# isarandi/metrabs

Hardware: AMD Instinct MI355X
Metric: crops/sec (256px, 72 depth bins) at 1/2/4/8 MI355X; MPJPE vs ref (higher is better)
Workload: dtype f32

## Files before the change

### include/metrabs_hip.h

```cpp
#ifndef METRABS_HIP_H_
#define METRABS_HIP_H_

#include <stddef.h>
#include <stdint.h>

#ifdef __cplusplus
extern "C" {
#endif

#define MTR_VERSION 100

typedef void* mtr_stream_t;

enum mtr_dtype { MTR_F32 = 0, MTR_F16 = 1, MTR_BF16 = 2 };

enum mtr_layout {
  MTR_NCHW = 0,
  MTR_NHWC = 1
};

enum mtr_error {
  MTR_OK = 0,
  MTR_E_NULL = -1,
  MTR_E_SHAPE = -2,
// ... 178 lines not shown
int mtr_bias_act_nchw(void* y, int dtype, const float* bias , const void* residual, int act,
                      long long B, int C, int HW, mtr_stream_t stream);

int mtr_bias_act_rowmean_nchw(void* y, int dtype, const float* bias , int act, long long B,
                              int C, int HW, float* row_mean , mtr_stream_t stream);

int mtr_depthwise3x3_bias_act(const void* x, int dtype, const float* weight, const float* bias, int act,
                              long long B, int C, int H, int W, int stride, int pad, void* y,
                              float* row_mean, mtr_stream_t stream);
int mtr_depthwise3x3_bias_act_padded(const void* x, int dtype, const float* weight, const float* bias,
                                     int act, long long B, int C, int H, int W, int stride, int pad_top,
                                     int pad_left, int pad_bottom, int pad_right, void* y,
                                     float* row_mean, mtr_stream_t stream);

int mtr_depthwise5x5_bias_act_padded(const void* x, int dtype, const float* weight ,
                                     const float* bias, int act, long long B, int C, int H, int W,
                                     int stride, int pad_top, int pad_left, int pad_bottom, int pad_right,
                                     void* y, float* row_mean , mtr_stream_t stream);

int mtr_se_gate(const float* mean , const float* w1, const float* b1, const float* w2,
                const float* b2, int act, int gate_fn, int B, int C, int S, float* gate ,
                mtr_stream_t stream);

int mtr_conv1x1_bias_act(const void* x, int dtype, const float* weight, const float* bias,
                         const float* gate , const void* residual, int act, long long B,
                         int M, int K, int HW, void* y, mtr_stream_t stream);

int mtr_conv1x1_bias_act16(const void* x, int dtype, const void* weight, const float* bias,
                           const float* gate , const void* residual, int act, long long B,
                           int M, int K, int HW, void* y, mtr_stream_t stream);

int mtr_conv3x3_bias_act16(const void* x, int dtype, const void* weight , const float* bias,
                           const void* residual, int act, long long B, int Cin, int Cout, int H, int W, int stride,
                           void* y, mtr_stream_t stream);

size_t mtr_conv3x3_16_lds_bytes(long long B, int Cin, int Cout, int H, int W, int stride);

#ifdef __cplusplus
}
#endif
#endif
```

### metrabs_amd/_lib.py

```python
import ctypes
import os
from ctypes import POINTER, c_char_p, c_double, c_float, c_int, c_int32, c_size_t, c_uint8, c_void_p

LIB_PATH = os.path.join(os.path.dirname(os.path.abspath(__file__)), 'csrc', 'libmetrabs_hip.so')

MTR_F32, MTR_F16, MTR_BF16 = 0, 1, 2
MTR_NCHW, MTR_NHWC = 0, 1
MTR_WARP_PARAM_FLOATS = 36


class HeadParams(ctypes.Structure):
    _fields_ = [('proc_side', c_int32), ('stride_test', c_int32), ('centered_stride', c_int32),
                ('legacy_centered_stride_bug', c_int32), ('box_size_mm', c_float)]


class HeadOptions(ctypes.Structure):
    _fields_ = [('struct_size', ctypes.c_uint32),
                ('rt_tiles_per_workgroup', c_int32), ('groups_per_workgroup', c_int32),
                ('dma_staging', c_int32), ('rt_column_blocks', c_int32), ('rt_k_groups', c_int32),
                ('rt_loader', c_int32), ('rt_split_column_blocks', c_int32)]


def head_options(rt_tiles=0, groups_per_workgroup=0, dma_staging=-1, rt_column_blocks=0, rt_k_groups=0,
                 rt_loader=0, rt_split=0):
# ... 92 lines not shown
    'mtr_detector_preprocess': (c_int, [c_void_p, c_int, c_int, c_int, POINTER(DetectorGeom), c_void_p,
                                        c_void_p]),
    'mtr_detector_preprocess_kernel': (c_int, [c_void_p, c_int, c_int, c_int, POINTER(DetectorGeom), c_int,
                                               c_void_p, c_void_p]),
    'mtr_detector_scale_boxes': (c_int, [c_void_p, c_int, POINTER(DetectorGeom), c_void_p, c_void_p]),
    'mtr_filter_poses_workspace_bytes': (ctypes.c_size_t, [c_int, c_int, c_int]),
    'mtr_filter_poses': (c_int, [c_void_p, c_void_p, c_void_p, c_void_p, c_void_p, c_int, c_int, c_int,
                                 c_int, c_void_p, c_void_p, c_int, c_int, POINTER(FilterParams), c_void_p,
                                 ctypes.c_size_t, c_int, c_void_p, c_void_p, c_void_p, c_void_p]),
    'mtr_depthwise3x3_bias_act': (c_int, [c_void_p, c_int, c_void_p, c_void_p, c_int, ctypes.c_longlong,
                                          c_int, c_int, c_int, c_int, c_int, c_void_p, c_void_p, c_void_p]),
    'mtr_depthwise3x3_bias_act_padded': (c_int, [c_void_p, c_int, c_void_p, c_void_p, c_int, ctypes.c_longlong,
                                                 c_int, c_int, c_int, c_int, c_int, c_int, c_int, c_int,
                                                 c_void_p, c_void_p, c_void_p]),
    'mtr_depthwise5x5_bias_act_padded': (c_int, [c_void_p, c_int, c_void_p, c_void_p, c_int, ctypes.c_longlong,
                                                 c_int, c_int, c_int, c_int, c_int, c_int, c_int, c_int,
                                                 c_void_p, c_void_p, c_void_p]),
    'mtr_bias_act_rowmean_nchw': (c_int, [c_void_p, c_int, c_void_p, c_int, ctypes.c_longlong, c_int, c_int,
                                          c_void_p, c_void_p]),
    'mtr_bias_act_nchw': (c_int, [c_void_p, c_int, c_void_p, c_void_p, c_int, ctypes.c_longlong, c_int,
                                  c_int, c_void_p]),
    'mtr_se_gate': (c_int, [c_void_p, c_void_p, c_void_p, c_void_p, c_void_p, c_int, c_int, c_int, c_int,
                            c_int, c_void_p, c_void_p]),
    'mtr_conv1x1_bias_act': (c_int, [c_void_p, c_int, c_void_p, c_void_p, c_void_p, c_void_p, c_int,
                                     ctypes.c_longlong, c_int, c_int, c_int, c_void_p, c_void_p]),
    'mtr_conv1x1_bias_act16': (c_int, [c_void_p, c_int, c_void_p, c_void_p, c_void_p, c_void_p, c_int,
                                       ctypes.c_longlong, c_int, c_int, c_int, c_void_p, c_void_p]),
    'mtr_conv3x3_bias_act16': (c_int, [c_void_p, c_int, c_void_p, c_void_p, c_void_p, c_int, ctypes.c_longlong,
                                       c_int, c_int, c_int, c_int, c_int, c_void_p, c_void_p]),
    'mtr_conv3x3_16_lds_bytes': (ctypes.c_size_t, [ctypes.c_longlong, c_int, c_int, c_int, c_int, c_int]),
}

_lib = None


def load(path=None):
    global _lib
    if _lib is not None and path is None:
        return _lib
    path = path or LIB_PATH
    import torch
    if not os.path.exists(path):
        raise RuntimeError(
            f'{path} not found: the HIP extension is not built. Run `python -m metrabs_amd.build` '
            f'(needs hipcc). metrabs_amd has no CPU fallback.')
    lib = ctypes.CDLL(path)
# ... 34 lines not shown
```

### metrabs_amd/backbones.py

```python
import collections
import threading

import torch
import torch.nn.functional as F
from torch import nn


class DepthwiseConv2d(nn.Conv2d):

    use_miopen = False
    _backend_lock = threading.Lock()

    def forward(self, x):
        if x.is_cuda and not DepthwiseConv2d.use_miopen and torch.backends.cudnn.enabled:
            cudnn = torch.backends.cudnn
            with DepthwiseConv2d._backend_lock, cudnn.flags(
                    enabled=False, benchmark=cudnn.benchmark, deterministic=cudnn.deterministic,
                    allow_tf32=cudnn.allow_tf32):
                return super().forward(x)
        return super().forward(x)


class ConvBNAct(nn.Sequential):

# ... 6 lines not shown
            layers.append(act())
        super().__init__(*layers)


class SqueezeExcite(nn.Module):
    def __init__(self, channels, squeeze, gate=nn.Sigmoid, act=nn.SiLU):
        super().__init__()
        self.fc1 = nn.Conv2d(channels, squeeze, 1)
        self.fc2 = nn.Conv2d(squeeze, channels, 1)
        self.act, self.gate = act(), gate()

    mean_from = ()
    gate_to = ()

    _GATE_NAMES = {nn.Sigmoid: 'sigmoid', nn.Hardsigmoid: 'hardsigmoid'}

    def forward(self, x):
        mean = None
        for src in self.mean_from:
            mean = src.take_mean_f32(x)
        if mean is not None and self._fused_gate_ok():
            from . import kernels
            g = kernels.se_gate(mean, self.fc1.weight, self.fc1.bias, self.fc2.weight, self.fc2.bias,
                                _ACT_NAMES[type(self.act)], self._GATE_NAMES[type(self.gate)])
            for dst in self.gate_to:
                if dst.k13_takes(x) or dst.k13h_takes(x):
                    dst.give_gate(x, g)
                    return x
            return x * g.to(x.dtype).view(x.shape[0], x.shape[1], 1, 1)
        if x.dtype != self.fc1.weight.dtype and not torch.is_autocast_enabled(x.device.type):
            return self._forward_16bit_copy(x, mean)
        s = None if mean is None else mean.to(x.dtype).view(x.shape[0], x.shape[1], 1, 1)
        if s is None:
            s = x.mean((2, 3), keepdim=True)
        return x * self.gate(self.fc2(self.act(self.fc1(s))))

    def _forward_16bit_copy(self, x, mean):
        s = mean.view(x.shape[0], x.shape[1], 1, 1) if mean is not None else \
            x.mean((2, 3), keepdim=True, dtype=self.fc1.weight.dtype)
        return x * self.gate(self.fc2(self.act(self.fc1(s)))).to(x.dtype)

    def _fused_gate_ok(self):
        if torch.is_grad_enabled() and any(p.requires_grad for p in self.parameters()):
            return False
        return (type(self.act) in (nn.SiLU, nn.ReLU) and type(self.gate) in self._GATE_NAMES
                and self.fc1.weight.dtype == torch.float32 and self.fc1.bias is not None
                and self.fc2.bias is not None and self.fc1.weight.is_cuda
                and self.fc1.in_channels % 4 == 0)


def _padded_conv(layers, name, cin, cout, k, stride, groups=1, act=nn.SiLU, bottomright=False):
    total = k - 1
    beg, end = total // 2, total - total // 2
    if bottomright:
        layers['padding'] = nn.ZeroPad2d((beg - 1, end + 1, beg - 1, end + 1))
        layers[name] = ConvBNAct(cin, cout, k, stride, groups=groups, act=act, padding=0)
    elif beg == end:
        layers[name] = ConvBNAct(cin, cout, k, stride, groups=groups, act=act, padding=beg)
    else:
        layers['padding'] = nn.ZeroPad2d((beg, end, beg, end))
        layers[name] = ConvBNAct(cin, cout, k, stride, groups=groups, act=act, padding=0)


# ... 136 lines not shown
        return resnet18()
    if name in ('mobilenetv3', 'mobilenetv3-large', 'mobilenet-v3'):
        return mobilenet_v3_large()
    raise ValueError(f'unknown backbone {name}')


_ACT_NAMES = {nn.SiLU: 'silu', nn.ReLU: 'relu', nn.Hardswish: 'hardswish'}


class ConvBiasAct(nn.Module):

    def __init__(self, conv, bias, act):
        super().__init__()
        self.conv = conv
        self.register_buffer('bias', bias.detach().float().contiguous())
        self.act = act
        self.act_name = None if act is None else _ACT_NAMES[type(act)]
        self.emit_mean = False
        self._mean = None
        self._gate = None
        self.last_path = None

    use_k13 = True
    k13_slower = frozenset({(960, 256, 64), (1536, 256, 64), (256, 1280, 64)})

    def k13_takes(self, x):
        c = self.conv
        if not (ConvBiasAct.use_k13 and not self.emit_mean and x.is_cuda and c.kernel_size == (1, 1)
                and c.stride == (1, 1) and c.padding == (0, 0) and c.dilation == (1, 1) and c.groups == 1
                and c.bias is None and c.padding_mode == 'zeros'):
            return False
        if torch.is_autocast_enabled('cuda') or (torch.is_grad_enabled() and c.weight.requires_grad):
            return False
        if x.dim() != 4 or (c.in_channels, c.out_channels, x.shape[2] * x.shape[3]) in ConvBiasAct.k13_slower:
            return False
        from . import kernels
        return kernels.conv1x1_supported(x, c.weight)

    use_k13h = True
    k13h_slower = frozenset({(192, 48, 4096), (256, 64, 1024), (1536, 256, 64), (256, 64, 9216), (768, 192, 576),
                             (1152, 224, 576), (1344, 224, 576), (1344, 384, 144), (2304, 384, 144),
                             (2304, 640, 144), (640, 3840, 144), (3840, 640, 144), (640, 1280, 144)})

    def k13h_takes(self, x):
        c = self.conv
        if not (ConvBiasAct.use_k13h and not self.emit_mean and x.is_cuda and x.dtype == c.weight.dtype
                and x.dtype in (torch.float16, torch.bfloat16) and c.kernel_size == (1, 1)
# ... 269 lines not shown
```

### metrabs_amd/csrc/conv1x1.hip

```cpp
#include "common.h"

namespace mtr {

typedef float f32x16 __attribute__((ext_vector_type(16)));

constexpr int kC1PadX = 32;
constexpr int kC1PadW = 4;

template <int WM, int WN, int FM, int FN, int BK, int ACT>
__global__ __launch_bounds__(64 * WM * WN) void conv1x1_kernel(
    const float* __restrict__ x, const float* __restrict__ w, const float* __restrict__ bias,
    const float* __restrict__ gate, const float* __restrict__ residual, float* __restrict__ y, int M,
    int K, int HW, int n_total, FastDiv by_hw) {
  constexpr int NT = 64 * WM * WN;
  constexpr int BM = 32 * FM * WM, BN = 32 * FN * WN;
  constexpr int LDX = BN + kC1PadX, LDW = BM + kC1PadW;
  constexpr int XROW4 = BN / 4;
  constexpr int XPASS = NT / XROW4;
  constexpr int XV = (BK + XPASS - 1) / XPASS;
  constexpr int WPASS = NT / (BK / 4);
  constexpr int WV = (BM + WPASS - 1) / WPASS;
  static_assert(NT % XROW4 == 0 && NT % (BK / 4) == 0, "loader mapping");
  __shared__ float xs[2][BK * LDX];
  __shared__ float ws[2][BK * LDW];
// ... 92 lines not shown
#pragma unroll
    for (int j = 0; j < FN; ++j) {
#pragma unroll
      for (int g = 0; g < 4; ++g) {
        const int col = n0 + wn * (32 * FN) + j * 32 + 8 * g + 4 * half;
        if (col >= n_total) continue;
        const unsigned b = fastdiv((unsigned)col, by_hw);
        const long long off = ((long long)b * M + m) * HW + (col - (int)b * HW);
        float4 r;
        r.x = activate<ACT>(acc[i][j][4 * g + 0] + bm);
        r.y = activate<ACT>(acc[i][j][4 * g + 1] + bm);
        r.z = activate<ACT>(acc[i][j][4 * g + 2] + bm);
        r.w = activate<ACT>(acc[i][j][4 * g + 3] + bm);
        if (residual) {
          const float4 q = *reinterpret_cast<const float4*>(residual + off);
          r.x += q.x; r.y += q.y; r.z += q.z; r.w += q.w;
        }
        *reinterpret_cast<float4*>(y + off) = r;
      }
    }
  }
}

enum Conv1x1Config { kCfgWide = 0, kCfgSquare = 1, kCfgTall = 2 };

struct Conv1x1Plan { int cfg, waves_m, bm, bn; };

inline Conv1x1Plan pick_config(int M, int K, int HW, long long B) {
  const long long n_total = B * HW;
  const long long n_tiles128 = (n_total + 127) / 128;
  if (M <= 160) {
    const int w = (M + 31) / 32;
    return {kCfgTall, w, 32 * w, 32};
  }
  if (M == 256 && K >= 512) return {kCfgTall, 4, 128, 32};
  if (M % 192 == 0 && (M / 192) * n_tiles128 >= 512) return {kCfgWide, 2, 192, 128};
  return {kCfgSquare, 2, 128, 128};
}

template <int WM, int WN, int FM, int FN, int BK>
static int launch_conv1x1_cfg(const float* x, const float* w, const float* bias, const float* gate,
                              const float* residual, float* y, int act, int M, int K, int HW,
                              long long n_total, hipStream_t stream) {
  constexpr int BM = 32 * FM * WM, BN = 32 * FN * WN;
  const long long gx = (n_total + BN - 1) / BN, gy = (M + BM - 1) / BM;
  if (gx > 0x7fffffffLL || gy > 65535) return MTR_E_SHAPE;
  const dim3 grid((unsigned)gx, (unsigned)gy), block(64 * WM * WN);
  const FastDiv by_hw = make_fastdiv((unsigned)HW);
  MTR_CLEAR_STALE();
#define MTR_C1_LAUNCH(ACT)                                                                                    \
  hipLaunchKernelGGL((conv1x1_kernel<WM, WN, FM, FN, BK, ACT>), grid, block, 0, stream, x, w, bias, gate, residual, \
                     y, M, K, HW, (int)n_total, by_hw)
  switch (act) {
    case kActNone: MTR_C1_LAUNCH(kActNone); break;
    case kActRelu: MTR_C1_LAUNCH(kActRelu); break;
    case kActSilu: MTR_C1_LAUNCH(kActSilu); break;
    case kActHardswish: MTR_C1_LAUNCH(kActHardswish); break;
    default: return MTR_E_PARAM;
  }
#undef MTR_C1_LAUNCH
  MTR_CHECK_LAUNCH();
  return MTR_OK;
}

}

extern "C" int mtr_conv1x1_bias_act(const void* x, int dtype, const float* weight, const float* bias,
                                    const float* gate, const void* residual, int act, long long B, int M,
                                    int K, int HW, void* y, mtr_stream_t stream) {
  if (!x || !weight || !bias || !y) return MTR_E_NULL;
  if (dtype != MTR_F32) return MTR_E_DTYPE;
  if (B < 0 || M <= 0 || K <= 0 || HW <= 0) return MTR_E_SHAPE;
  if (HW % 4 || K % 4) return MTR_E_SHAPE;
  if (B * HW > 0x7fffffffLL || (long long)K * HW > 0x7fffffffLL || (long long)M * HW > 0x7fffffffLL)
    return MTR_E_SHAPE;
  if (act < mtr::kActNone || act > mtr::kActHardswish) return MTR_E_PARAM;
  if (((uintptr_t)x % 16) || ((uintptr_t)weight % 16) || ((uintptr_t)y % 16) || ((uintptr_t)residual % 16))
    return MTR_E_ALIGN;
  if (x == y || (residual && residual == x)) return MTR_E_PARAM;
  if (B == 0) return MTR_OK;
  const float* xf = (const float*)x;
  const float* rf = (const float*)residual;
  float* yf = (float*)y;
  const long long n_total = B * HW;
  hipStream_t s = (hipStream_t)stream;
  const mtr::Conv1x1Plan p = mtr::pick_config(M, K, HW, B);
  switch (p.cfg) {
    case mtr::kCfgWide:
      return mtr::launch_conv1x1_cfg<2, 2, 3, 2, 16>(xf, weight, bias, gate, rf, yf, act, M, K, HW, n_total, s);
    case mtr::kCfgSquare:
      return mtr::launch_conv1x1_cfg<2, 2, 2, 2, 16>(xf, weight, bias, gate, rf, yf, act, M, K, HW, n_total, s);
    default:
      switch (p.waves_m) {
        case 1: return mtr::launch_conv1x1_cfg<1, 1, 1, 1, 16>(xf, weight, bias, gate, rf, yf, act, M, K, HW, n_total, s);
        case 2: return mtr::launch_conv1x1_cfg<2, 1, 1, 1, 16>(xf, weight, bias, gate, rf, yf, act, M, K, HW, n_total, s);
        case 3: return mtr::launch_conv1x1_cfg<3, 1, 1, 1, 16>(xf, weight, bias, gate, rf, yf, act, M, K, HW, n_total, s);
        case 4: return mtr::launch_conv1x1_cfg<4, 1, 1, 1, 32>(xf, weight, bias, gate, rf, yf, act, M, K, HW, n_total, s);
        default: return mtr::launch_conv1x1_cfg<5, 1, 1, 1, 16>(xf, weight, bias, gate, rf, yf, act, M, K, HW, n_total, s);
      }
  }
}
```

### metrabs_amd/csrc/se.hip

```cpp
#include "common.h"

namespace mtr {

enum SeGate { kGateSigmoid = 0, kGateHardsigmoid = 1 };

constexpr int kSeThreads = 256;
constexpr int kSeImg = 4;
constexpr int kSeRows = 4;
constexpr int kSeUnroll = 4;

template <int ACT, int GATE>
__global__ __launch_bounds__(kSeThreads) void se_gate_kernel(const float* __restrict__ mean,
                                                             const float* __restrict__ w1,
                                                             const float* __restrict__ b1,
                                                             const float* __restrict__ w2,
                                                             const float* __restrict__ b2, int B,
                                                             int C, int S, float* __restrict__ gate) {
  extern __shared__ float4 se_lds[];
  const int C4 = C >> 2;
  float4* m_tile = se_lds;
  float* hid = reinterpret_cast<float*>(se_lds + kSeImg * C4);
  const int b0 = blockIdx.y * kSeImg;
  const int tid = threadIdx.x, lane = tid & 63, wave = tid >> 6;

  for (int i = tid; i < kSeImg * C4; i += kSeThreads) {
    const int img = i / C4, c4 = i - img * C4;
    m_tile[i] = b0 + img < B ? reinterpret_cast<const float4*>(mean)[(long long)(b0 + img) * C4 + c4]
                             : make_float4(0.0f, 0.0f, 0.0f, 0.0f);
  }
  __syncthreads();

  const int n_blocks = (S + kSeRows - 1) / kSeRows;
  for (int blk = wave; blk < n_blocks; blk += kSeThreads / 64) {
    const float4* wrow[kSeRows];
#pragma unroll
    for (int r = 0; r < kSeRows; ++r) {
      const int s = min(blk * kSeRows + r, S - 1);
      wrow[r] = reinterpret_cast<const float4*>(w1 + (long long)s * C);
    }
    float acc[kSeRows][kSeImg];
#pragma unroll
    for (int r = 0; r < kSeRows; ++r)
#pragma unroll
      for (int i = 0; i < kSeImg; ++i) acc[r][i] = 0.0f;
    for (int c0 = lane; c0 < C4; c0 += 64 * kSeUnroll) {
      float4 w[kSeUnroll][kSeRows];
#pragma unroll
      for (int u = 0; u < kSeUnroll; ++u)
#pragma unroll
        for (int r = 0; r < kSeRows; ++r)
          w[u][r] = wrow[r][min(c0 + 64 * u, C4 - 1)];
#pragma unroll
      for (int u = 0; u < kSeUnroll; ++u) {
        const int c4 = c0 + 64 * u;
        const bool live = c4 < C4;
        float4 m[kSeImg];
#pragma unroll
        for (int i = 0; i < kSeImg; ++i) {
          const float4 v = m_tile[i * C4 + min(c4, C4 - 1)];
          m[i] = live ? v : make_float4(0.0f, 0.0f, 0.0f, 0.0f);
        }
#pragma unroll
        for (int r = 0; r < kSeRows; ++r)
#pragma unroll
          for (int i = 0; i < kSeImg; ++i) {
            float a = acc[r][i];
            a = fmaf(w[u][r].x, m[i].x, a);
            a = fmaf(w[u][r].y, m[i].y, a);
            a = fmaf(w[u][r].z, m[i].z, a);
            a = fmaf(w[u][r].w, m[i].w, a);
            acc[r][i] = a;
          }
      }
    }
#pragma unroll
    for (int r = 0; r < kSeRows; ++r)
#pragma unroll
      for (int i = 0; i < kSeImg; ++i) {
        float v = acc[r][i];
#pragma unroll
        for (int k = 32; k >= 1; k >>= 1) v += __shfl_xor(v, k, 64);
        acc[r][i] = v;
      }
    if (lane == 0) {
#pragma unroll
      for (int r = 0; r < kSeRows; ++r) {
        const int s = blk * kSeRows + r;
        if (s < S) {
#pragma unroll
          for (int i = 0; i < kSeImg; ++i) hid[i * S + s] = activate<ACT>(acc[r][i] + b1[s]);
        }
      }
    }
  }
  __syncthreads();

  const int c = blockIdx.x * kSeThreads + tid;
  if (c >= C) return;
  const float* w2row = w2 + (long long)c * S;
  float z[kSeImg];
#pragma unroll
  for (int i = 0; i < kSeImg; ++i) z[i] = 0.0f;
#pragma unroll 16
  for (int s = 0; s < S; ++s) {
    const float w = w2row[s];
#pragma unroll
    for (int i = 0; i < kSeImg; ++i) z[i] = fmaf(w, hid[i * S + s], z[i]);
  }
  const float bias = b2[c];
#pragma unroll
  for (int i = 0; i < kSeImg; ++i) {
    if (b0 + i >= B) break;
    const float x = z[i] + bias;
    float g;
    if constexpr (GATE == kGateSigmoid) g = 1.0f / (1.0f + expf(-x));
    else g = fminf(fmaxf(x + 3.0f, 0.0f), 6.0f) / 6.0f;
    gate[(long long)(b0 + i) * C + c] = g;
  }
}

template <int ACT>
static int launch_se_gate(const float* mean, const float* w1, const float* b1, const float* w2,
                          const float* b2, int gate_fn, int B, int C, int S, float* gate,
                          hipStream_t stream) {
  const size_t lds = (size_t)kSeImg * C * sizeof(float) + (size_t)kSeImg * S * sizeof(float);
  const dim3 grid((C + kSeThreads - 1) / kSeThreads, (B + kSeImg - 1) / kSeImg), block(kSeThreads);
  const void* kern = gate_fn == kGateSigmoid ? (const void*)se_gate_kernel<ACT, kGateSigmoid>
                                             : (const void*)se_gate_kernel<ACT, kGateHardsigmoid>;
  if (lds > 64 * 1024) {
    const int e = allow_dynamic_lds(kern, lds);
    if (e != MTR_OK) return e;
  }
  MTR_CLEAR_STALE();
  if (gate_fn == kGateSigmoid)
    hipLaunchKernelGGL((se_gate_kernel<ACT, kGateSigmoid>), grid, block, lds, stream, mean, w1, b1, w2, b2,
                       B, C, S, gate);
  else
    hipLaunchKernelGGL((se_gate_kernel<ACT, kGateHardsigmoid>), grid, block, lds, stream, mean, w1, b1, w2,
                       b2, B, C, S, gate);
  MTR_CHECK_LAUNCH();
  return MTR_OK;
}

}

extern "C" int mtr_se_gate(const float* mean, const float* w1, const float* b1, const float* w2,
                           const float* b2, int act, int gate_fn, int B, int C, int S, float* gate,
                           mtr_stream_t stream) {
  if (!mean || !w1 || !b1 || !w2 || !b2 || !gate) return MTR_E_NULL;
  if (B < 0 || C <= 0 || S <= 0 || C % 4 || (B + mtr::kSeImg - 1) / mtr::kSeImg > 65535) return MTR_E_SHAPE;
  if ((long long)mtr::kSeImg * (C + S) * 4 > 160 * 1024) return MTR_E_SHAPE;
  if (((uintptr_t)mean % 16) || ((uintptr_t)w1 % 16)) return MTR_E_ALIGN;
  if (gate_fn != mtr::kGateSigmoid && gate_fn != mtr::kGateHardsigmoid) return MTR_E_PARAM;
  if (B == 0) return MTR_OK;
  hipStream_t s = (hipStream_t)stream;
  switch (act) {
    case mtr::kActNone: return mtr::launch_se_gate<mtr::kActNone>(mean, w1, b1, w2, b2, gate_fn, B, C, S, gate, s);
    case mtr::kActRelu: return mtr::launch_se_gate<mtr::kActRelu>(mean, w1, b1, w2, b2, gate_fn, B, C, S, gate, s);
    case mtr::kActSilu: return mtr::launch_se_gate<mtr::kActSilu>(mean, w1, b1, w2, b2, gate_fn, B, C, S, gate, s);
    case mtr::kActHardswish: return mtr::launch_se_gate<mtr::kActHardswish>(mean, w1, b1, w2, b2, gate_fn, B, C, S, gate, s);
    default: return MTR_E_PARAM;
  }
}
```

### metrabs_amd/kernels.py

```python
import ctypes

import torch

from metrabs_amd import _lib
from metrabs_amd._lib import check, current_stream_ptr, dtype_code, require_cuda


def _ptr(t):
    return ctypes.c_void_p(t.data_ptr()) if t is not None else ctypes.c_void_p(0)


def softargmax_decode(logits, n_points, cfg, out=None, nhwc_staging=0):
    require_cuda(logits)
    lib = _lib.load()
    nhwc = _is_channels_last(logits)
    if not nhwc:
        logits = logits.contiguous()
    B, n_out, H, W = logits.shape
    J = int(n_points)
    D = n_out // J - 1
    if n_out != J * (1 + D) or D != cfg.depth:
        raise ValueError(f'logits have {n_out} channels, expected J*(1+depth) = {J * (1 + cfg.depth)}')
    if out is None:
        c2d = torch.empty(B, J, 2, device=logits.device, dtype=torch.float32)
# ... 491 lines not shown

def depthwise5x5_bias_act(x, weight, bias, act, stride, pad, want_mean=False):
    require_cuda(x, weight, bias)
    if not x.is_contiguous():
        raise ValueError('depthwise5x5_bias_act needs an NCHW-contiguous tensor')
    if weight.numel() != x.shape[1] * 25:
        raise ValueError(f'depthwise5x5_bias_act needs a [C, 5, 5] weight, got {tuple(weight.shape)}')
    B, C, H, W = x.shape
    pl, pr, pt, pb = (pad,) * 4 if isinstance(pad, int) else tuple(int(p) for p in pad)
    OH, OW = (H + pt + pb - 5) // stride + 1, (W + pl + pr - 5) // stride + 1
    y = torch.empty(B, C, max(OH, 0), max(OW, 0), device=x.device, dtype=x.dtype)
    mean = torch.empty(B, C, device=x.device, dtype=torch.float32) if want_mean else None
    check(_lib.load().mtr_depthwise5x5_bias_act_padded(
        _ptr(x), dtype_code(x.dtype), _ptr(weight.contiguous().float()), _ptr(bias.contiguous().float()),
        ACT_CODES[act], B, C, H, W, int(stride), pt, pl, pb, pr, _ptr(y), None if mean is None else _ptr(mean),
        current_stream_ptr(x.device)), 'mtr_depthwise5x5_bias_act_padded')
    return (y, mean) if want_mean else y



SE_GATE_CODES = {'sigmoid': 0, 'hardsigmoid': 1}


def se_gate(mean, w1, b1, w2, b2, act, gate_fn, out=None):
    require_cuda(mean, w1, b1, w2, b2)
    B, C = mean.shape[0], mean.shape[1]
    S = w1.shape[0]
    w1, w2 = w1.reshape(S, -1), w2.reshape(C, -1)
    if mean.dtype != torch.float32 or mean.numel() != B * C or w1.shape[1] != C or w2.shape[1] != S:
        raise ValueError('se_gate: mean [B, C] f32, w1 [S, C], w2 [C, S]')
    tensors = [t.contiguous().float() for t in (mean, w1, b1, w2, b2)]
    if out is None:
        out = torch.empty(B, C, device=mean.device, dtype=torch.float32)
    check(_lib.load().mtr_se_gate(*(_ptr(t) for t in tensors), ACT_CODES[act], SE_GATE_CODES[gate_fn], B, C, S,
                                  _ptr(out), current_stream_ptr(mean.device)), 'mtr_se_gate')
    return out



def conv1x1_supported(x, weight):
    if x.dim() != 4 or x.dtype != torch.float32 or weight.dtype != torch.float32 or not x.is_contiguous():
        return False
    K, HW = x.shape[1], x.shape[2] * x.shape[3]
    return (weight.numel() == weight.shape[0] * K and HW % 4 == 0 and K % 4 == 0
            and x.data_ptr() % 16 == 0 and weight.data_ptr() % 16 == 0
            and x.shape[0] * HW < 2 ** 31 and K * HW < 2 ** 31 and weight.shape[0] * HW < 2 ** 31)


def conv1x1_bias_act(x, w, bias, act, gate=None, residual=None, out=None):
    require_cuda(x, w, bias, gate, residual)
    B, K, H, W = x.shape
    M = w.shape[0]
    w = w.reshape(M, -1)
    if w.shape[1] != K:
        raise ValueError(f'conv1x1_bias_act: weight has {w.shape[1]} input channels, x has {K}')
    if gate is not None and (gate.dtype != torch.float32 or gate.numel() != B * K):
        raise ValueError('conv1x1_bias_act: gate must be [B, Cin] f32')
    if residual is not None and (residual.shape != (B, M, H, W) or residual.dtype != x.dtype
                                 or not residual.is_contiguous()):
        raise ValueError('conv1x1_bias_act: residual must be [B, Cout, H, W] like the output, contiguous')
    if out is None:
        out = torch.empty(B, M, H, W, device=x.device, dtype=x.dtype)
    elif out.shape != (B, M, H, W) or out.dtype != x.dtype or not out.is_contiguous():
        raise ValueError('conv1x1_bias_act: out must be [B, Cout, H, W] like the output, contiguous')
    check(_lib.load().mtr_conv1x1_bias_act(
        _ptr(x), dtype_code(x.dtype), _ptr(w.contiguous()), _ptr(bias.contiguous().float()),
        None if gate is None else _ptr(gate.contiguous()), None if residual is None else _ptr(residual),
        ACT_CODES[act], B, M, K, H * W, _ptr(out), current_stream_ptr(x.device)), 'mtr_conv1x1_bias_act')
    return out



def conv1x1_16_supported(x, weight):
    if x.dim() != 4 or x.dtype not in (torch.float16, torch.bfloat16) or weight.dtype != x.dtype \
            or not x.is_contiguous() or not weight.is_contiguous():
        return False
    K, HW = x.shape[1], x.shape[2] * x.shape[3]
    return (weight.numel() == weight.shape[0] * K and HW % 8 == 0 and K % 8 == 0
            and x.data_ptr() % 16 == 0 and weight.data_ptr() % 16 == 0
            and x.shape[0] * HW < 2 ** 31 and K * HW < 2 ** 31 and weight.shape[0] * HW < 2 ** 31)


def conv1x1_bias_act16(x, w, bias, act, gate=None, residual=None, out=None):
    require_cuda(x, w, bias, gate, residual)
    B, K, H, W = x.shape
    M = w.shape[0]
    w = w.reshape(M, -1)
    if w.shape[1] != K:
        raise ValueError(f'conv1x1_bias_act16: weight has {w.shape[1]} input channels, x has {K}')
    if w.dtype != x.dtype:
        raise ValueError(f'conv1x1_bias_act16: weight is {w.dtype}, x is {x.dtype}')
# ... 62 lines not shown
```

Before: 8377.

## Add deep-K MFMA conv1x1 path and retuned SE gate kernel with transposed fc2

Adds a new f32 conv1x1 kernel for small spatial, deep-K shapes that uses a narrow N tile, a 3-stage LDS pipeline and MFMA 16x16x4 f32 instructions. It is selected automatically for M=256, K>=512, HW<=64, and for large-M small-K cases that now route to the tall config. The SE gate kernel is reworked to use 1024 threads with configurable images-per-block and a cached transposed fc2 weight for coalesced reads. The k13 exclusion list is shrunk so more layers take the fused k13 path. These aim to improve occupancy and memory coalescing for low-resolution layers, at the cost of new code paths that may be slower for some shapes.

```diff
diff --git a/include/metrabs_hip.h b/include/metrabs_hip.h
--- a/include/metrabs_hip.h
+++ b/include/metrabs_hip.h
@@ -224,9 +224,21 @@
                 const float* b2, int act, int gate_fn, int B, int C, int S, float* gate ,
                 mtr_stream_t stream);
 
+#define MTR_SE_W2_CS 0
+#define MTR_SE_W2_SC 1
+int mtr_se_gate_opts(const float* mean , const float* w1, const float* b1, const float* w2,
+                     const float* b2, int act, int gate_fn, int B, int C, int S, float* gate ,
+                     mtr_stream_t stream, int w2_layout, int config);
+
 int mtr_conv1x1_bias_act(const void* x, int dtype, const float* weight, const float* bias,
                          const float* gate , const void* residual, int act, long long B,
                          int M, int K, int HW, void* y, mtr_stream_t stream);
+
+int mtr_conv1x1_bias_act_opts(const void* x, int dtype, const float* weight, const float* bias,
+                              const float* gate , const void* residual, int act, long long B,
+                              int M, int K, int HW, void* y, mtr_stream_t stream, int config);
+
+int mtr_conv1x1_plan(int M, int K, int HW, long long B, int config, int* plan );
 
 int mtr_conv1x1_bias_act16(const void* x, int dtype, const void* weight, const float* bias,
                            const float* gate , const void* residual, int act, long long B,
diff --git a/metrabs_amd/_lib.py b/metrabs_amd/_lib.py
--- a/metrabs_amd/_lib.py
+++ b/metrabs_amd/_lib.py
@@ -138,6 +138,11 @@
                                   c_int, c_void_p]),
     'mtr_se_gate': (c_int, [c_void_p, c_void_p, c_void_p, c_void_p, c_void_p, c_int, c_int, c_int, c_int,
                             c_int, c_void_p, c_void_p]),
+    'mtr_se_gate_opts': (c_int, [c_void_p, c_void_p, c_void_p, c_void_p, c_void_p, c_int, c_int, c_int, c_int,
+                                 c_int, c_void_p, c_void_p, c_int, c_int]),
+    'mtr_conv1x1_bias_act_opts': (c_int, [c_void_p, c_int, c_void_p, c_void_p, c_void_p, c_void_p, c_int,
+                                          ctypes.c_longlong, c_int, c_int, c_int, c_void_p, c_void_p, c_int]),
+    'mtr_conv1x1_plan': (c_int, [c_int, c_int, c_int, ctypes.c_longlong, c_int, c_void_p]),
     'mtr_conv1x1_bias_act': (c_int, [c_void_p, c_int, c_void_p, c_void_p, c_void_p, c_void_p, c_int,
                                      ctypes.c_longlong, c_int, c_int, c_int, c_void_p, c_void_p]),
     'mtr_conv1x1_bias_act16': (c_int, [c_void_p, c_int, c_void_p, c_void_p, c_void_p, c_void_p, c_int,
diff --git a/metrabs_amd/backbones.py b/metrabs_amd/backbones.py
--- a/metrabs_amd/backbones.py
+++ b/metrabs_amd/backbones.py
@@ -52,7 +52,7 @@
         if mean is not None and self._fused_gate_ok():
             from . import kernels
             g = kernels.se_gate(mean, self.fc1.weight, self.fc1.bias, self.fc2.weight, self.fc2.bias,
-                                _ACT_NAMES[type(self.act)], self._GATE_NAMES[type(self.gate)])
+                                _ACT_NAMES[type(self.act)], self._GATE_NAMES[type(self.gate)], w2t=self._fc2_wt())
             for dst in self.gate_to:
                 if dst.k13_takes(x) or dst.k13h_takes(x):
                     dst.give_gate(x, g)
@@ -69,6 +69,15 @@
         s = mean.view(x.shape[0], x.shape[1], 1, 1) if mean is not None else \
             x.mean((2, 3), keepdim=True, dtype=self.fc1.weight.dtype)
         return x * self.gate(self.fc2(self.act(self.fc1(s)))).to(x.dtype)
+
+    _w2t = None
+
+    def _fc2_wt(self):
+        w = self.fc2.weight
+        key = (w.data_ptr(), w.device, None if w.is_inference() else w._version)
+        if self._w2t is None or self._w2t[0] != key:
+            self._w2t = (key, w.detach().reshape(w.shape[0], -1).t().contiguous())
+        return self._w2t[1]
 
     def _fused_gate_ok(self):
         if torch.is_grad_enabled() and any(p.requires_grad for p in self.parameters()):
@@ -251,7 +260,7 @@
         self.last_path = None
 
     use_k13 = True
-    k13_slower = frozenset({(960, 256, 64), (1536, 256, 64), (256, 1280, 64)})
+    k13_slower = frozenset({(1536, 256, 64)})
 
     def k13_takes(self, x):
         c = self.conv
diff --git a/metrabs_amd/csrc/conv1x1.hip b/metrabs_amd/csrc/conv1x1.hip
--- a/metrabs_amd/csrc/conv1x1.hip
+++ b/metrabs_amd/csrc/conv1x1.hip
@@ -1,3 +1,5 @@
+#include <type_traits>
+
 #include "common.h"
 
 namespace mtr {
@@ -138,20 +140,189 @@
   }
 }
 
-enum Conv1x1Config { kCfgWide = 0, kCfgSquare = 1, kCfgTall = 2 };
+constexpr int kDkBK = 32, kDkBN = 16, kDkStages = 3;
+constexpr int kDkLDW = kDkBK + 4;
+
+typedef float f32x4 __attribute__((ext_vector_type(4)));
+
+constexpr size_t deepk_lds_bytes(int waves) {
+  return (size_t)kDkStages * (kDkBK * kDkBN + 32 * waves * kDkLDW) * sizeof(float);
+}
+
+template <int WAVES, int ACT>
+__global__ __launch_bounds__(64 * WAVES) void conv1x1_deepk_kernel(
+    const float* __restrict__ x, const float* __restrict__ w, const float* __restrict__ bias,
+    const float* __restrict__ gate, const float* __restrict__ residual, float* __restrict__ y, int M,
+    int K, int HW, int n_total, FastDiv by_hw) {
+  constexpr int NT = 64 * WAVES, BM = 32 * WAVES;
+  constexpr int XS = kDkBK * kDkBN, WS = BM * kDkLDW;
+  static_assert(BM * (kDkBK / 4) == 4 * NT, "W loader mapping");
+  extern __shared__ float4 dk_lds[];
+  float* xs = reinterpret_cast<float*>(dk_lds);
+  float* ws = xs + kDkStages * XS;
+
+  const int tid = threadIdx.x, lane = tid & 63, wave = tid >> 6;
+  const int m0 = blockIdx.y * BM, n0 = blockIdx.x * kDkBN;
+  const long long khw = (long long)K * HW;
+
+  constexpr int XV = XS / NT;
+  static_assert(XV * NT == XS && (XV == 1 || XV == 2), "x loader mapping");
+  const int xp = (tid % (kDkBN / XV)) * XV, xk = tid / (kDkBN / XV);
+  const int xcol = n0 + xp;
+  const bool xcol_ok = xcol < n_total;
+  const unsigned xb = xcol_ok ? fastdiv((unsigned)xcol, by_hw) : 0u;
+  const float* xsrc = xcol_ok ? x + (long long)xb * khw + (xcol - (int)xb * HW) : x;
+  const bool has_gate = gate != nullptr;
+  const float* gsrc = has_gate ? gate + (long long)xb * K : x;
+  const int wk4 = tid & 7, wr0 = tid >> 3;
+
+  const float4 zero = make_float4(0.0f, 0.0f, 0.0f, 0.0f);
+  float4 rw[2][4] = {{zero, zero, zero, zero}, {zero, zero, zero, zero}};
+  float rx[2][XV] = {}, rg[2] = {1.0f, 1.0f};
+  auto load_tile = [&](int kt, auto set) {
+    constexpr int P = decltype(set)::value;
+    const int k0 = kt * kDkBK;
+    const int kx = min(k0 + xk, K - 1);
+    if constexpr (XV == 2) {
+      const float2 t = *reinterpret_cast<const float2*>(xsrc + (long long)kx * HW);
+      rx[P][0] = t.x; rx[P][XV - 1] = t.y;
+    } else {
+      rx[P][0] = xsrc[(long long)kx * HW];
+    }
+    rg[P] = gsrc[kx];
+    const int k = min(k0 + wk4 * 4, K - 4);
+#pragma unroll
+    for (int v = 0; v < 4; ++v) {
+      const int m = min(m0 + wr0 + v * (NT / 8), M - 1);
+      rw[P][v] = *reinterpret_cast<const float4*>(w + (long long)m * K + k);
+    }
+  };
+  auto store_tile = [&](int stage, int kt, auto set) {
+    constexpr int P = decltype(set)::value;
+    const int k0 = kt * kDkBK;
+    const float g = has_gate ? rg[P] : 1.0f;
+    const bool x_ok = xcol_ok && k0 + xk < K;
+    float* xd = &xs[stage * XS + xk * kDkBN + xp];
+    if constexpr (XV == 2) {
+      *reinterpret_cast<float2*>(xd) = make_float2(x_ok ? rx[P][0] * g : 0.0f, x_ok ? rx[P][XV - 1] * g : 0.0f);
+    } else {
+      *xd = x_ok ? rx[P][0] * g : 0.0f;
+    }
+    const bool k_ok = k0 + wk4 * 4 < K;
+#pragma unroll
+    for (int v = 0; v < 4; ++v) {
+      const int row = wr0 + v * (NT / 8);
+      const bool ok = k_ok && m0 + row < M;
+      float4 u = rw[P][v];
+      u.x = ok ? u.x : 0.0f; u.y = ok ? u.y : 0.0f; u.z = ok ? u.z : 0.0f; u.w = ok ? u.w : 0.0f;
+      *reinterpret_cast<float4*>(&ws[stage * WS + row * kDkLDW + wk4 * 4]) = u;
+    }
+  };
+
+  f32x4 acc[2];
+#pragma unroll
+  for (int f = 0; f < 2; ++f)
+#pragma unroll
+    for (int r = 0; r < 4; ++r) acc[f][r] = 0.0f;
+
+  const int c = lane & 15, kg = lane >> 4;
+  auto multiply = [&](int stage, int kk0) {
+    const float* xb_ = &xs[stage * XS + kg * kDkBN + c];
+    const float* wb_ = &ws[stage * WS + (wave * 32 + c) * kDkLDW + kg];
+#pragma unroll
+    for (int kk = kk0; kk < kk0 + kDkBK / 2; kk += 4) {
+      const float a = xb_[kk * kDkBN];
+      const float b0 = wb_[kk], b1 = wb_[16 * kDkLDW + kk];
+      acc[0] = __builtin_amdgcn_mfma_f32_16x16x4f32(a, b0, acc[0], 0, 0, 0);
+      acc[1] = __builtin_amdgcn_mfma_f32_16x16x4f32(a, b1, acc[1], 0, 0, 0);
+    }
+  };
+
+  const int n_tiles = (K + kDkBK - 1) / kDkBK;
+  constexpr std::integral_constant<int, 0> ra{};
+  constexpr std::integral_constant<int, 1> rb{};
+  load_tile(0, ra);
+  if (n_tiles > 1) load_tile(1, rb);
+  store_tile(0, 0, ra);
+  if (n_tiles > 1) store_tile(1, 1, rb);
+  if (n_tiles > 2) load_tile(2, ra);
+  __syncthreads();
+  int stage = 0;
+  auto step = [&](int t, auto hold, auto issue, auto guarded) {
+    constexpr bool G = decltype(guarded)::value;
+    if (!G || t + 3 < n_tiles) load_tile(t + 3, issue);
+    multiply(stage, 0);
+    __builtin_amdgcn_sched_barrier(0);
+    if (!G || t + 2 < n_tiles) store_tile(stage == 0 ? 2 : stage - 1, t + 2, hold);
+    __builtin_amdgcn_sched_barrier(0);
+    multiply(stage, kDkBK / 2);
+    stage = stage == 2 ? 0 : stage + 1;
+    __syncthreads();
+  };
+  int t = 0;
+  for (; t + 4 < n_tiles; t += 2) {
+    step(t, ra, rb, std::false_type{});
+    step(t + 1, rb, ra, std::false_type{});
+  }
+  for (; t < n_tiles; t += 2) {
+    step(t, ra, rb, std::true_type{});
+    if (t + 1 < n_tiles) step(t + 1, rb, ra, std::true_type{});
+  }
+
+  const int col = n0 + 4 * kg;
+  if (col >= n_total) return;
+  const unsigned b = fastdiv((unsigned)col, by_hw);
+#pragma unroll
+  for (int f = 0; f < 2; ++f) {
+    const int m = m0 + wave * 32 + f * 16 + c;
+    if (m >= M) continue;
+    const float bm = bias[m];
+    const long long off = ((long long)b * M + m) * HW + (col - (int)b * HW);
+    float4 r;
+    r.x = activate<ACT>(acc[f][0] + bm);
+    r.y = activate<ACT>(acc[f][1] + bm);
+    r.z = activate<ACT>(acc[f][2] + bm);
+    r.w = activate<ACT>(acc[f][3] + bm);
+    if (residual) {
+      const float4 q = *reinterpret_cast<const float4*>(residual + off);
+      r.x += q.x; r.y += q.y; r.z += q.z; r.w += q.w;
+    }
+    *reinterpret_cast<float4*>(y + off) = r;
+  }
+}
+
+enum Conv1x1Config { kCfgWide = 0, kCfgSquare = 1, kCfgTall = 2, kCfgDeepK = 3, kCfgCount = 4 };
 
 struct Conv1x1Plan { int cfg, waves_m, bm, bn; };
+
+inline Conv1x1Plan plan_tall(int M) {
+  const int w = M <= 160 ? (M + 31) / 32 : 4;
+  return {kCfgTall, w, 32 * w, 32};
+}
+inline Conv1x1Plan plan_deepk(int M) {
+  const int w = M <= 128 ? 4 : 8;
+  return {kCfgDeepK, w, 32 * w, kDkBN};
+}
 
 inline Conv1x1Plan pick_config(int M, int K, int HW, long long B) {
   const long long n_total = B * HW;
   const long long n_tiles128 = (n_total + 127) / 128;
-  if (M <= 160) {
-    const int w = (M + 31) / 32;
-    return {kCfgTall, w, 32 * w, 32};
-  }
-  if (M == 256 && K >= 512) return {kCfgTall, 4, 128, 32};
+  if (M <= 160) return plan_tall(M);
+  if (M == 256 && K >= 512) return HW <= 64 ? plan_deepk(M) : plan_tall(M);
+  if (M >= 1024 && M % 128 == 0 && K <= 256 && n_tiles128 <= 32) return plan_tall(M);
   if (M % 192 == 0 && (M / 192) * n_tiles128 >= 512) return {kCfgWide, 2, 192, 128};
   return {kCfgSquare, 2, 128, 128};
+}
+
+inline int plan_for(int M, int K, int HW, long long B, int config, Conv1x1Plan* p) {
+  switch (config) {
+    case -1: *p = pick_config(M, K, HW, B); return MTR_OK;
+    case kCfgWide: *p = {kCfgWide, 2, 192, 128}; return MTR_OK;
+    case kCfgSquare: *p = {kCfgSquare, 2, 128, 128}; return MTR_OK;
+    case kCfgTall: *p = plan_tall(M); return MTR_OK;
+    case kCfgDeepK: *p = plan_deepk(M); return MTR_OK;
+    default: return MTR_E_PARAM;
+  }
 }
 
 template <int WM, int WN, int FM, int FN, int BK>
@@ -179,11 +350,59 @@
   return MTR_OK;
 }
 
+template <int WAVES>
+static int launch_conv1x1_deepk(const float* x, const float* w, const float* bias, const float* gate,
+                                const float* residual, float* y, int act, int M, int K, int HW,
+                                long long n_total, hipStream_t stream) {
+  constexpr int BM = 32 * WAVES;
+  constexpr size_t lds = deepk_lds_bytes(WAVES);
+  const long long gx = (n_total + kDkBN - 1) / kDkBN, gy = (M + BM - 1) / BM;
+  if (gx > 0x7fffffffLL || gy > 65535) return MTR_E_SHAPE;
+  const dim3 grid((unsigned)gx, (unsigned)gy), block(64 * WAVES);
+  const FastDiv by_hw = make_fastdiv((unsigned)HW);
+#define MTR_DK_LAUNCH(ACT)                                                                                 \
+  do {                                                                                                     \
+    if (lds > 64 * 1024) {                                                                                 \
+      const int e = allow_dynamic_lds((const void*)conv1x1_deepk_kernel<WAVES, ACT>, lds);                 \
+      if (e != MTR_OK) return e;                                                                           \
+    }                                                                                                      \
+    MTR_CLEAR_STALE();                                                                                     \
+    hipLaunchKernelGGL((conv1x1_deepk_kernel<WAVES, ACT>), grid, block, lds, stream, x, w, bias, gate,     \
+                       residual, y, M, K, HW, (int)n_total, by_hw);                                        \
+  } while (0)
+  switch (act) {
+    case kActNone: MTR_DK_LAUNCH(kActNone); break;
+    case kActRelu: MTR_DK_LAUNCH(kActRelu); break;
+    case kActSilu: MTR_DK_LAUNCH(kActSilu); break;
+    case kActHardswish: MTR_DK_LAUNCH(kActHardswish); break;
+    default: return MTR_E_PARAM;
+  }
+#undef MTR_DK_LAUNCH
+  MTR_CHECK_LAUNCH();
+  return MTR_OK;
+}
+
+}
+
+extern "C" int mtr_conv1x1_plan(int M, int K, int HW, long long B, int config, int* plan) {
+  if (!plan) return MTR_E_NULL;
+  if (B < 0 || M <= 0 || K <= 0 || HW <= 0) return MTR_E_SHAPE;
+  mtr::Conv1x1Plan p;
+  const int e = mtr::plan_for(M, K, HW, B, config, &p);
+  if (e != MTR_OK) return e;
+  plan[0] = p.cfg; plan[1] = p.waves_m; plan[2] = p.bm; plan[3] = p.bn;
+  return MTR_OK;
 }
 
 extern "C" int mtr_conv1x1_bias_act(const void* x, int dtype, const float* weight, const float* bias,
                                     const float* gate, const void* residual, int act, long long B, int M,
                                     int K, int HW, void* y, mtr_stream_t stream) {
+  return mtr_conv1x1_bias_act_opts(x, dtype, weight, bias, gate, residual, act, B, M, K, HW, y, stream, -1);
+}
+
+extern "C" int mtr_conv1x1_bias_act_opts(const void* x, int dtype, const float* weight, const float* bias,
+                                         const float* gate, const void* residual, int act, long long B,
+                                         int M, int K, int HW, void* y, mtr_stream_t stream, int config) {
   if (!x || !weight || !bias || !y) return MTR_E_NULL;
   if (dtype != MTR_F32) return MTR_E_DTYPE;
   if (B < 0 || M <= 0 || K <= 0 || HW <= 0) return MTR_E_SHAPE;
@@ -200,12 +419,18 @@
   float* yf = (float*)y;
   const long long n_total = B * HW;
   hipStream_t s = (hipStream_t)stream;
-  const mtr::Conv1x1Plan p = mtr::pick_config(M, K, HW, B);
+  mtr::Conv1x1Plan p;
+  if (mtr::plan_for(M, K, HW, B, config, &p) != MTR_OK) return MTR_E_PARAM;
   switch (p.cfg) {
     case mtr::kCfgWide:
       return mtr::launch_conv1x1_cfg<2, 2, 3, 2, 16>(xf, weight, bias, gate, rf, yf, act, M, K, HW, n_total, s);
     case mtr::kCfgSquare:
       return mtr::launch_conv1x1_cfg<2, 2, 2, 2, 16>(xf, weight, bias, gate, rf, yf, act, M, K, HW, n_total, s);
+    case mtr::kCfgDeepK:
+      switch (p.waves_m) {
+        case 4: return mtr::launch_conv1x1_deepk<4>(xf, weight, bias, gate, rf, yf, act, M, K, HW, n_total, s);
+        default: return mtr::launch_conv1x1_deepk<8>(xf, weight, bias, gate, rf, yf, act, M, K, HW, n_total, s);
+      }
     default:
       switch (p.waves_m) {
         case 1: return mtr::launch_conv1x1_cfg<1, 1, 1, 1, 16>(xf, weight, bias, gate, rf, yf, act, M, K, HW, n_total, s);
diff --git a/metrabs_amd/csrc/se.hip b/metrabs_amd/csrc/se.hip
--- a/metrabs_amd/csrc/se.hip
+++ b/metrabs_amd/csrc/se.hip
@@ -4,26 +4,29 @@
 
 enum SeGate { kGateSigmoid = 0, kGateHardsigmoid = 1 };
 
-constexpr int kSeThreads = 256;
+constexpr int kSeThreads = 1024;
 constexpr int kSeImg = 4;
-constexpr int kSeRows = 4;
-constexpr int kSeUnroll = 4;
 
-template <int ACT, int GATE>
+template <int IMG, int IPT, bool W2T>
 __global__ __launch_bounds__(kSeThreads) void se_gate_kernel(const float* __restrict__ mean,
                                                              const float* __restrict__ w1,
                                                              const float* __restrict__ b1,
                                                              const float* __restrict__ w2,
-                                                             const float* __restrict__ b2, int B,
-                                                             int C, int S, float* __restrict__ gate) {
+                                                             const float* __restrict__ b2, int act,
+                                                             int gate_fn, int B, int C, int S,
+                                                             float* __restrict__ gate) {
+  constexpr int kSeRows = IMG <= 4 ? 4 : 2;
+  constexpr int kSeUnroll = IMG <= 4 ? 2 : 1;
+  static_assert(IMG % IPT == 0 && kSeThreads % (IMG / IPT) == 0, "thread mapping");
+  constexpr int CS = kSeThreads / (IMG / IPT);
   extern __shared__ float4 se_lds[];
   const int C4 = C >> 2;
   float4* m_tile = se_lds;
-  float* hid = reinterpret_cast<float*>(se_lds + kSeImg * C4);
-  const int b0 = blockIdx.y * kSeImg;
+  float* hid = reinterpret_cast<float*>(se_lds + IMG * C4);
+  const int b0 = blockIdx.y * IMG;
   const int tid = threadIdx.x, lane = tid & 63, wave = tid >> 6;
 
-  for (int i = tid; i < kSeImg * C4; i += kSeThreads) {
+  for (int i = tid; i < IMG * C4; i += kSeThreads) {
     const int img = i / C4, c4 = i - img * C4;
     m_tile[i] = b0 + img < B ? reinterpret_cast<const float4*>(mean)[(long long)(b0 + img) * C4 + c4]
                              : make_float4(0.0f, 0.0f, 0.0f, 0.0f);
@@ -38,127 +41,159 @@
       const int s = min(blk * kSeRows + r, S - 1);
       wrow[r] = reinterpret_cast<const float4*>(w1 + (long long)s * C);
     }
-    float acc[kSeRows][kSeImg];
+    float acc[kSeRows][IMG];
 #pragma unroll
     for (int r = 0; r < kSeRows; ++r)
 #pragma unroll
-      for (int i = 0; i < kSeImg; ++i) acc[r][i] = 0.0f;
-    for (int c0 = lane; c0 < C4; c0 += 64 * kSeUnroll) {
+      for (int i = 0; i < IMG; ++i) acc[r][i] = 0.0f;
+    for (int cb = 0; cb < C4; cb += 64 * kSeUnroll) {
       float4 w[kSeUnroll][kSeRows];
 #pragma unroll
-      for (int u = 0; u < kSeUnroll; ++u)
+      for (int u = 0; u < kSeUnroll; ++u) {
+        if (cb + 64 * u < C4) {
 #pragma unroll
-        for (int r = 0; r < kSeRows; ++r)
-          w[u][r] = wrow[r][min(c0 + 64 * u, C4 - 1)];
+          for (int r = 0; r < kSeRows; ++r) w[u][r] = wrow[r][min(cb + 64 * u + lane, C4 - 1)];
+        } else {
+#pragma unroll
+          for (int r = 0; r < kSeRows; ++r) w[u][r] = make_float4(0.0f, 0.0f, 0.0f, 0.0f);
+        }
+      }
 #pragma unroll
       for (int u = 0; u < kSeUnroll; ++u) {
-        const int c4 = c0 + 64 * u;
+        const int c4 = cb + 64 * u + lane;
         const bool live = c4 < C4;
-        float4 m[kSeImg];
 #pragma unroll
-        for (int i = 0; i < kSeImg; ++i) {
+        for (int i = 0; i < IMG; ++i) {
           const float4 v = m_tile[i * C4 + min(c4, C4 - 1)];
-          m[i] = live ? v : make_float4(0.0f, 0.0f, 0.0f, 0.0f);
-        }
+          const float4 m = live ? v : make_float4(0.0f, 0.0f, 0.0f, 0.0f);
 #pragma unroll
-        for (int r = 0; r < kSeRows; ++r)
-#pragma unroll
-          for (int i = 0; i < kSeImg; ++i) {
+          for (int r = 0; r < kSeRows; ++r) {
             float a = acc[r][i];
-            a = fmaf(w[u][r].x, m[i].x, a);
-            a = fmaf(w[u][r].y, m[i].y, a);
-            a = fmaf(w[u][r].z, m[i].z, a);
-            a = fmaf(w[u][r].w, m[i].w, a);
+            a = fmaf(w[u][r].x, m.x, a);
+            a = fmaf(w[u][r].y, m.y, a);
+            a = fmaf(w[u][r].z, m.z, a);
+            a = fmaf(w[u][r].w, m.w, a);
             acc[r][i] = a;
           }
+        }
       }
     }
+    float mine = 0.0f;
 #pragma unroll
     for (int r = 0; r < kSeRows; ++r)
 #pragma unroll
-      for (int i = 0; i < kSeImg; ++i) {
+      for (int i = 0; i < IMG; ++i) {
         float v = acc[r][i];
 #pragma unroll
         for (int k = 32; k >= 1; k >>= 1) v += __shfl_xor(v, k, 64);
-        acc[r][i] = v;
+        mine = lane == r * IMG + i ? v : mine;
       }
-    if (lane == 0) {
-#pragma unroll
-      for (int r = 0; r < kSeRows; ++r) {
-        const int s = blk * kSeRows + r;
-        if (s < S) {
-#pragma unroll
-          for (int i = 0; i < kSeImg; ++i) hid[i * S + s] = activate<ACT>(acc[r][i] + b1[s]);
-        }
-      }
+    const int s = blk * kSeRows + lane / IMG;
+    if (lane < kSeRows * IMG && s < S) {
+      const float h = mine + b1[s];
+      float a = h;
+      if (act == kActRelu) a = activate<kActRelu>(h);
+      else if (act == kActSilu) a = activate<kActSilu>(h);
+      else if (act == kActHardswish) a = activate<kActHardswish>(h);
+      hid[(lane % IMG) * S + s] = a;
     }
   }
   __syncthreads();
 
-  const int c = blockIdx.x * kSeThreads + tid;
+  const int isub = tid / CS;
+  const int c = blockIdx.x * CS + (tid - isub * CS);
   if (c >= C) return;
-  const float* w2row = w2 + (long long)c * S;
-  float z[kSeImg];
+  const float* hrow = hid + isub * IPT * S;
+  const float* wsrc = W2T ? w2 + c : w2 + (long long)c * S;
+  const long long wstep = W2T ? C : 1;
+  float z[IPT];
 #pragma unroll
-  for (int i = 0; i < kSeImg; ++i) z[i] = 0.0f;
+  for (int i = 0; i < IPT; ++i) z[i] = 0.0f;
 #pragma unroll 16
   for (int s = 0; s < S; ++s) {
-    const float w = w2row[s];
+    const float w = wsrc[s * wstep];
 #pragma unroll
-    for (int i = 0; i < kSeImg; ++i) z[i] = fmaf(w, hid[i * S + s], z[i]);
+    for (int i = 0; i < IPT; ++i) z[i] = fmaf(w, hrow[i * S + s], z[i]);
   }
   const float bias = b2[c];
 #pragma unroll
-  for (int i = 0; i < kSeImg; ++i) {
-    if (b0 + i >= B) break;
+  for (int i = 0; i < IPT; ++i) {
+    const int b = b0 + isub * IPT + i;
+    if (b >= B) break;
     const float x = z[i] + bias;
     float g;
-    if constexpr (GATE == kGateSigmoid) g = 1.0f / (1.0f + expf(-x));
+    if (gate_fn == kGateSigmoid) g = 1.0f / (1.0f + expf(-x));
     else g = fminf(fmaxf(x + 3.0f, 0.0f), 6.0f) / 6.0f;
-    gate[(long long)(b0 + i) * C + c] = g;
+    gate[(long long)b * C + c] = g;
   }
 }
 
-template <int ACT>
+constexpr int kSeConfigs = 4;
+
+inline size_t se_lds_bytes(int img, int C, int S) { return (size_t)img * ((size_t)C + S) * sizeof(float); }
+
+inline int se_pick_config(int B, int C, int S) {
+  const long long groups2 = ((long long)B + 1) / 2, slices2 = (C + 511) / 512;
+  const long long w1_reread = groups2 * slices2 * S * C * 4;
+  if (groups2 <= 65535 && w1_reread <= 64ll << 20) return 3;
+  return 1;
+}
+
+template <int IMG, int IPT, bool W2T>
 static int launch_se_gate(const float* mean, const float* w1, const float* b1, const float* w2,
-                          const float* b2, int gate_fn, int B, int C, int S, float* gate,
+                          const float* b2, int act, int gate_fn, int B, int C, int S, float* gate,
                           hipStream_t stream) {
-  const size_t lds = (size_t)kSeImg * C * sizeof(float) + (size_t)kSeImg * S * sizeof(float);
-  const dim3 grid((C + kSeThreads - 1) / kSeThreads, (B + kSeImg - 1) / kSeImg), block(kSeThreads);
-  const void* kern = gate_fn == kGateSigmoid ? (const void*)se_gate_kernel<ACT, kGateSigmoid>
-                                             : (const void*)se_gate_kernel<ACT, kGateHardsigmoid>;
+  constexpr int CS = kSeThreads / (IMG / IPT);
+  const size_t lds = se_lds_bytes(IMG, C, S);
+  const int gy = (B + IMG - 1) / IMG;
+  if (gy > 65535 || lds > 160 * 1024) return MTR_E_SHAPE;
+  const dim3 grid((C + CS - 1) / CS, gy), block(kSeThreads);
   if (lds > 64 * 1024) {
-    const int e = allow_dynamic_lds(kern, lds);
+    const int e = allow_dynamic_lds((const void*)se_gate_kernel<IMG, IPT, W2T>, lds);
     if (e != MTR_OK) return e;
   }
   MTR_CLEAR_STALE();
-  if (gate_fn == kGateSigmoid)
-    hipLaunchKernelGGL((se_gate_kernel<ACT, kGateSigmoid>), grid, block, lds, stream, mean, w1, b1, w2, b2,
-                       B, C, S, gate);
-  else
-    hipLaunchKernelGGL((se_gate_kernel<ACT, kGateHardsigmoid>), grid, block, lds, stream, mean, w1, b1, w2,
-                       b2, B, C, S, gate);
+  hipLaunchKernelGGL((se_gate_kernel<IMG, IPT, W2T>), grid, block, lds, stream, mean, w1, b1, w2, b2, act,
+                     gate_fn, B, C, S, gate);
   MTR_CHECK_LAUNCH();
   return MTR_OK;
 }
 
+template <bool W2T>
+static int launch_se_gate_cfg(int config, const float* mean, const float* w1, const float* b1,
+                              const float* w2, const float* b2, int act, int gate_fn, int B, int C, int S,
+                              float* gate, hipStream_t stream) {
+  switch (config) {
+    case 0: return launch_se_gate<4, 1, W2T>(mean, w1, b1, w2, b2, act, gate_fn, B, C, S, gate, stream);
+    case 1: return launch_se_gate<4, 4, W2T>(mean, w1, b1, w2, b2, act, gate_fn, B, C, S, gate, stream);
+    case 2: return launch_se_gate<8, 2, W2T>(mean, w1, b1, w2, b2, act, gate_fn, B, C, S, gate, stream);
+    default: return launch_se_gate<2, 1, W2T>(mean, w1, b1, w2, b2, act, gate_fn, B, C, S, gate, stream);
+  }
+}
+
+}
+
+extern "C" int mtr_se_gate_opts(const float* mean, const float* w1, const float* b1, const float* w2,
+                                const float* b2, int act, int gate_fn, int B, int C, int S, float* gate,
+                                mtr_stream_t stream, int w2_layout, int config) {
+  if (!mean || !w1 || !b1 || !w2 || !b2 || !gate) return MTR_E_NULL;
+  if (B < 0 || C <= 0 || S <= 0 || C % 4 || (B + mtr::kSeImg - 1) / mtr::kSeImg > 65535) return MTR_E_SHAPE;
+  if ((long long)mtr::kSeImg * (C + S) * 4 > 160 * 1024) return MTR_E_SHAPE;
+  if (((uintptr_t)mean % 16) || ((uintptr_t)w1 % 16)) return MTR_E_ALIGN;
+  if (gate_fn != mtr::kGateSigmoid && gate_fn != mtr::kGateHardsigmoid) return MTR_E_PARAM;
+  if (act < mtr::kActNone || act > mtr::kActHardswish) return MTR_E_PARAM;
+  if (w2_layout != MTR_SE_W2_CS && w2_layout != MTR_SE_W2_SC) return MTR_E_PARAM;
+  if (config < -1 || config >= mtr::kSeConfigs) return MTR_E_PARAM;
+  if (B == 0) return MTR_OK;
+  if (config < 0) config = mtr::se_pick_config(B, C, S);
+  hipStream_t s = (hipStream_t)stream;
+  if (w2_layout == MTR_SE_W2_SC)
+    return mtr::launch_se_gate_cfg<true>(config, mean, w1, b1, w2, b2, act, gate_fn, B, C, S, gate, s);
+  return mtr::launch_se_gate_cfg<false>(config, mean, w1, b1, w2, b2, act, gate_fn, B, C, S, gate, s);
 }
 
 extern "C" int mtr_se_gate(const float* mean, const float* w1, const float* b1, const float* w2,
                            const float* b2, int act, int gate_fn, int B, int C, int S, float* gate,
                            mtr_stream_t stream) {
-  if (!mean || !w1 || !b1 || !w2 || !b2 || !gate) return MTR_E_NULL;
-  if (B < 0 || C <= 0 || S <= 0 || C % 4 || (B + mtr::kSeImg - 1) / mtr::kSeImg > 65535) return MTR_E_SHAPE;
-  if ((long long)mtr::kSeImg * (C + S) * 4 > 160 * 1024) return MTR_E_SHAPE;
-  if (((uintptr_t)mean % 16) || ((uintptr_t)w1 % 16)) return MTR_E_ALIGN;
-  if (gate_fn != mtr::kGateSigmoid && gate_fn != mtr::kGateHardsigmoid) return MTR_E_PARAM;
-  if (B == 0) return MTR_OK;
-  hipStream_t s = (hipStream_t)stream;
-  switch (act) {
-    case mtr::kActNone: return mtr::launch_se_gate<mtr::kActNone>(mean, w1, b1, w2, b2, gate_fn, B, C, S, gate, s);
-    case mtr::kActRelu: return mtr::launch_se_gate<mtr::kActRelu>(mean, w1, b1, w2, b2, gate_fn, B, C, S, gate, s);
-    case mtr::kActSilu: return mtr::launch_se_gate<mtr::kActSilu>(mean, w1, b1, w2, b2, gate_fn, B, C, S, gate, s);
-    case mtr::kActHardswish: return mtr::launch_se_gate<mtr::kActHardswish>(mean, w1, b1, w2, b2, gate_fn, B, C, S, gate, s);
-    default: return MTR_E_PARAM;
-  }
+  return mtr_se_gate_opts(mean, w1, b1, w2, b2, act, gate_fn, B, C, S, gate, stream, MTR_SE_W2_CS, -1);
 }
diff --git a/metrabs_amd/kernels.py b/metrabs_amd/kernels.py
--- a/metrabs_amd/kernels.py
+++ b/metrabs_amd/kernels.py
@@ -537,18 +537,23 @@
 SE_GATE_CODES = {'sigmoid': 0, 'hardsigmoid': 1}
 
 
-def se_gate(mean, w1, b1, w2, b2, act, gate_fn, out=None):
-    require_cuda(mean, w1, b1, w2, b2)
+def se_gate(mean, w1, b1, w2, b2, act, gate_fn, out=None, w2t=None, config=-1):
+    require_cuda(mean, w1, b1, w2, b2, w2t)
     B, C = mean.shape[0], mean.shape[1]
     S = w1.shape[0]
     w1, w2 = w1.reshape(S, -1), w2.reshape(C, -1)
     if mean.dtype != torch.float32 or mean.numel() != B * C or w1.shape[1] != C or w2.shape[1] != S:
         raise ValueError('se_gate: mean [B, C] f32, w1 [S, C], w2 [C, S]')
+    if w2t is not None:
+        if w2t.shape != (S, C) or w2t.dtype != torch.float32 or not w2t.is_contiguous():
+            raise ValueError('se_gate: w2t must be [S, C] f32, contiguous')
+        w2 = w2t
     tensors = [t.contiguous().float() for t in (mean, w1, b1, w2, b2)]
     if out is None:
         out = torch.empty(B, C, device=mean.device, dtype=torch.float32)
-    check(_lib.load().mtr_se_gate(*(_ptr(t) for t in tensors), ACT_CODES[act], SE_GATE_CODES[gate_fn], B, C, S,
-                                  _ptr(out), current_stream_ptr(mean.device)), 'mtr_se_gate')
+    check(_lib.load().mtr_se_gate_opts(*(_ptr(t) for t in tensors), ACT_CODES[act], SE_GATE_CODES[gate_fn], B, C,
+                                       S, _ptr(out), current_stream_ptr(mean.device),
+                                       0 if w2t is None else 1, int(config)), 'mtr_se_gate_opts')
     return out
 
 
@@ -562,7 +567,19 @@
             and x.shape[0] * HW < 2 ** 31 and K * HW < 2 ** 31 and weight.shape[0] * HW < 2 ** 31)
 
 
-def conv1x1_bias_act(x, w, bias, act, gate=None, residual=None, out=None):
+CONV1X1_CONFIGS = {'auto': -1, 'wide': 0, 'square': 1, 'tall': 2, 'deepk': 3}
+
+
+def conv1x1_plan(M, K, HW, B, config='auto'):
+    import ctypes
+    plan = (ctypes.c_int * 4)()
+    check(_lib.load().mtr_conv1x1_plan(M, K, HW, B, CONV1X1_CONFIGS[config], ctypes.addressof(plan)),
+          'mtr_conv1x1_plan')
+    names = {v: k for k, v in CONV1X1_CONFIGS.items()}
+    return names[plan[0]], plan[1], plan[2], plan[3]
+
+
+def conv1x1_bias_act(x, w, bias, act, gate=None, residual=None, out=None, config='auto'):
     require_cuda(x, w, bias, gate, residual)
     B, K, H, W = x.shape
     M = w.shape[0]
@@ -578,10 +595,11 @@
         out = torch.empty(B, M, H, W, device=x.device, dtype=x.dtype)
     elif out.shape != (B, M, H, W) or out.dtype != x.dtype or not out.is_contiguous():
         raise ValueError('conv1x1_bias_act: out must be [B, Cout, H, W] like the output, contiguous')
-    check(_lib.load().mtr_conv1x1_bias_act(
+    check(_lib.load().mtr_conv1x1_bias_act_opts(
         _ptr(x), dtype_code(x.dtype), _ptr(w.contiguous()), _ptr(bias.contiguous().float()),
         None if gate is None else _ptr(gate.contiguous()), None if residual is None else _ptr(residual),
-        ACT_CODES[act], B, M, K, H * W, _ptr(out), current_stream_ptr(x.device)), 'mtr_conv1x1_bias_act')
+        ACT_CODES[act], B, M, K, H * W, _ptr(out), current_stream_ptr(x.device), CONV1X1_CONFIGS[config]),
+        'mtr_conv1x1_bias_act_opts')
     return out
 
 
```

Result: faster. 8744, median of 6 (+4.4%).
